# rteammco/super-resolution

Measured on AMD Instinct MI355X. Metric: MAP gradient iterations/sec at fixed HR size, higher is better.
Workload: dtype f64

## Files before the change

super-resolution_amd/csrc/kernels_ztile.hip:

```cpp


#include <type_traits>

#include "ztile_dev.hpp"

namespace srmap {

namespace {

template <typename T, int S, int B, int REGK, int R, bool WD, bool SP>
__global__ __launch_bounds__((ZCfg<T, S, B, REGK, R>::NT), (sizeof(T) == 4 || S == 2 ? 6 : 4)) void k_eval_z(
    ZArgs<T, B, ZCfg<T, S, B, REGK, R>::NP> A) {
  using C = ZCfg<T, S, B, REGK, R>;
  constexpr int HB = C::HB, NV = C::NV, RU = C::RU;
  constexpr int kBorderLds = (int)((16 * sizeof(int2) + kBorderTabEntries * sizeof(ZEntry) + 16 * sizeof(double) + sizeof(T) - 1) / sizeof(T));
  __shared__ T xs[C::XS_ELEMS > kBorderLds ? C::XS_ELEMS : kBorderLds];
  __shared__ T zs[C::ZS_ELEMS > 0 ? C::ZS_ELEMS : 1];
  __shared__ T cs[C::CS_ELEMS > 0 ? C::CS_ELEMS : 1];
  __shared__ double red[2][C::NW];
  __shared__ T wcs[32];
  __shared__ T whs[(C::RU > 0 ? C::RU : 1) * S * C::CW];

  {
    const T* a_x = A.x; const T* a_y = A.y; const T* a_w = A.w; T* a_g = A.g;
// ... 15 lines not shown
      if (WD && A.fold_xk != nullptr) border_block<T, S, B, C::NT, WD, WD>(A, Bd, bidx, blockIdx.z, xs, A.nby * gridDim.x);
      else border_block<T, S, B, C::NT, WD, false>(A, Bd, bidx, blockIdx.z, xs, A.nby * gridDim.x);
    }
    else if (threadIdx.x == 0) {
      const int nbb = A.nby * gridDim.x;
      put_partial<WD>(A, (size_t)A.n_tile_partials + (size_t)blockIdx.z * nbb + bidx, 0.0, 0.0);
    }
    return;
  }
  const int by = blockIdx.y - A.nby, nby_t = gridDim.y - A.nby;
  int tby = by, tbx = blockIdx.x;
  {
    const int q = gridDim.x >> 3, rem = gridDim.x & 7;
    const int n0 = blockIdx.x, nbot = (rem == 0) ? (int)gridDim.x - 1 : 8 * q - 1;
    const int n = (nbot > 1) ? (n0 == 1 ? nbot : (n0 == nbot ? 1 : n0)) : n0;
    const int bnd = n & 7;
    tby = bnd * q + (bnd < rem ? bnd : rem) + (n >> 3);
    tbx = (by == 0) ? 0 : (by == 1 ? nby_t - 1 : by - 1);
  }
  if (A.sel_mode != 0 && ((A.sel_mode == 1) != (tby >= A.sel0 && tby < A.sel1))) return;
  const int R0 = tby * C::TH, CJ0 = tbx * C::CW, C0 = CJ0 * S;
  const int ch = blockIdx.z;
  const size_t N = (size_t)A.W * A.H;
  const size_t nl = (size_t)A.wl * A.hl;
  const bool fold = WD && A.fold_xk != nullptr;
  const T* xplane = (fold ? A.fold_xk : A.x) + (size_t)ch * N;
  const int gr = R0 + wv;
  const int gc0 = C0 + S * lane;
  const int cellg = CJ0 + lane;
  const bool want_data = (A.terms & SRMAP_TERM_DATA) != 0;
  const bool want_reg = REGK != 0 && (A.terms & SRMAP_TERM_REG) != 0 && R0 >= A.rr0 && R0 < A.rr1;
  const T* ybase = A.y + (size_t)ch * nl;
  constexpr int ARI = (C::XR + C::NW - 1) / C::NW;
  constexpr int EXTRA = C::XC - C::CW;
  constexpr bool XT = ARI >= 2 && (C::NW - 1) + (ARI - 1) * C::NW >= C::XR && C::XR * EXTRA <= 64;
  T va[ARI][S], vb[ARI][S], ma[ARI], mb[ARI];
  T vda[WD ? ARI : 1][S], vdb[WD ? ARI : 1][S];
  bool owna[ARI] = {}, ownb[ARI] = {};
  size_t xoa[ARI] = {}, xob[ARI] = {};
#pragma unroll
  for (int it = 0; it < ARI; ++it) {
    const bool xt_slot = XT && it == ARI - 1 && wv == C::NW - 1;
    const int row = xt_slot ? lane / EXTRA : wv + it * C::NW;
    const int grr = R0 - C::HU + row;
    const bool row_in = row < C::XR && (unsigned)grr < (unsigned)A.H;
    const int gca = xt_slot ? CJ0 - C::XCL + C::CW + lane % EXTRA : CJ0 - C::XCL + lane, gcb = gca + C::CW;
    const bool ina = row_in && (unsigned)gca < (unsigned)A.wl;
    const bool inb = !XT && row_in && lane < EXTRA && (unsigned)gcb < (unsigned)A.wl;
    const T* sa = xplane + (ina ? (size_t)grr * A.W + (size_t)gca * S : (size_t)0);
    const T* sb = xplane + (inb ? (size_t)grr * A.W + (size_t)gcb * S : (size_t)0);
#pragma unroll
    for (int pc = 0; pc < S; ++pc) va[it][pc] = sa[pc];
    if (!XT) {
#pragma unroll
      for (int pc = 0; pc < S; ++pc) vb[it][pc] = sb[pc];
    }
    if (WD) {
#pragma unroll
      for (int pc = 0; pc < S; ++pc) { vda[it][pc] = T(0); vdb[it][pc] = T(0); }
      if (fold) {
        const T* dpl = A.dvec + (size_t)ch * N;
        const T* da = dpl + (sa - xplane);
        const T* db = dpl + (sb - xplane);
#pragma unroll
        for (int pc = 0; pc < S; ++pc) vda[it][pc] = da[pc];
        if (!XT) {
#pragma unroll
          for (int pc = 0; pc < S; ++pc) vdb[it][pc] = db[pc];
        }
        const int orow = row - C::HU;
        owna[it] = ina && orow >= 0 && orow < C::TH && gca >= CJ0 && gca < CJ0 + C::CW;
        ownb[it] = inb && orow >= 0 && orow < C::TH && gcb >= CJ0 && gcb < CJ0 + C::CW;
        xoa[it] = (size_t)grr * A.W + (size_t)gca * S;
        xob[it] = (size_t)grr * A.W + (size_t)gcb * S;
      }
    }
    ma[it] = ina ? Pre<T>::up(T(1)) : T(0);
    mb[it] = inb ? Pre<T>::up(T(1)) : T(0);
  }
  T ypre[NV];
#pragma unroll
  for (int v = 0; v < NV; ++v) ypre[v] = T(0);
  const int rm = A.E + HB + 1, cm = (A.E + HB + S) / S + 1;
  const bool edge = (R0 - rm < 0) || (R0 + C::TH + rm > A.H) || (CJ0 - cm < 0) || (CJ0 + C::CW + cm > A.wl) ||
                    A.cr0 > 0 || A.cr1 < A.H;
  const int hrowz = wv == 0 ? -HB : C::TH - 1 + HB;
  const bool has_z_halo = want_data && B > 1 && A.g != nullptr && wv < 2;
  T ypre2[NV];
#pragma unroll
  for (int v = 0; v < NV; ++v) ypre2[v] = T(0);
  if (!SP && want_data) z_row_prefetch<T, S, B, C>(A, wv, R0, CJ0, lane, edge, ybase, ypre);
  if (!SP && has_z_halo) z_row_prefetch<T, S, B, C>(A, hrowz, R0, CJ0, lane, edge, ybase, ypre2);
  const T* wplane = (want_reg && A.w) ? A.w + (size_t)ch * N : nullptr;
  T wreg[S];
#pragma unroll
  for (int pc = 0; pc < S; ++pc) wreg[pc] = T(1);
  if (wplane != nullptr && gr < A.H && gc0 < A.W) {
#pragma unroll
    for (int pc = 0; pc < S; ++pc) wreg[pc] = wplane[(size_t)gr * A.W + gc0 + pc];
  }
  const bool reg_halo_on = want_reg && A.g != nullptr && RU > 0;
  const int hrow = -(wv - 1);
  const bool has_reg_halo = reg_halo_on && wv >= 2 && wv < 2 + RU;
  T whalo[S];
#pragma unroll
  for (int pc = 0; pc < S; ++pc) whalo[pc] = T(1);
  if (has_reg_halo && wplane != nullptr && R0 + hrow >= 0 && gc0 < A.W) {
#pragma unroll
    for (int pc = 0; pc < S; ++pc) whalo[pc] = wplane[(size_t)(R0 + hrow) * A.W + gc0 + pc];
  }

  T wcolv = T(1);
  const bool col_task = reg_halo_on && (wv == 4 || wv == 5) && lane < C::TH + RU;
  if (col_task && wplane != nullptr) {
    const int hgr = R0 + lane - RU, hgc = C0 - (wv == 4 ? 1 : 2);
    if (hgr >= 0 && hgr < A.H && hgc >= 0) wcolv = wplane[(size_t)hgr * A.W + hgc];
  }

  const DirScale dsc = dir_scale(WD ? A.fold_norms : nullptr);
  if (WD && fold) {
    T* xout = A.fold_x + (size_t)ch * N;
#pragma unroll
    for (int it = 0; it < ARI; ++it) {
#pragma unroll
      for (int pc = 0; pc < S; ++pc) va[it][pc] = va[it][pc] + A.fold_stp * dir_elem<T>(vda[it][pc], dsc);
      if (owna[it]) {
#pragma unroll
        for (int pc = 0; pc < S; ++pc) xout[xoa[it] + pc] = va[it][pc];
      }
      if (!XT) {
#pragma unroll
        for (int pc = 0; pc < S; ++pc) vb[it][pc] = vb[it][pc] + A.fold_stp * dir_elem<T>(vdb[it][pc], dsc);
        if (ownb[it]) {
#pragma unroll
          for (int pc = 0; pc < S; ++pc) xout[xob[it] + pc] = vb[it][pc];
        }
      }
    }
  }
#pragma unroll
  for (int it = 0; it < ARI; ++it) {
    const bool xt_slot = XT && it == ARI - 1 && wv == C::NW - 1;
    if (xt_slot) {
      const int xrow = lane / EXTRA;
      if (xrow < C::XR) {
#pragma unroll
        for (int pc = 0; pc < S; ++pc) xs[xrow * C::XROW + pc * C::XC + C::CW + lane % EXTRA] = va[it][pc] * ma[it];
      }
      continue;
    }
    const int row = wv + it * C::NW;
    if (row < C::XR) {
#pragma unroll
      for (int pc = 0; pc < S; ++pc) xs[row * C::XROW + pc * C::XC + lane] = va[it][pc] * ma[it];
      if (!XT && lane < EXTRA) {
#pragma unroll
        for (int pc = 0; pc < S; ++pc) xs[row * C::XROW + pc * C::XC + C::CW + lane] = vb[it][pc] * mb[it];
      }
    }
  }
  if (col_task) wcs[(wv - 4) * 16 + lane] = wcolv;
  if (has_reg_halo) {
#pragma unroll
    for (int pc = 0; pc < S; ++pc) whs[((wv - 2) * S + pc) * C::CW + lane] = whalo[pc];
  }
  __syncthreads();

  T mk[S];
#pragma unroll
  for (int pc = 0; pc < S; ++pc) mk[pc] = (gr < A.H && gc0 + pc < A.W) ? T(1) : T(0);

  T acc[S], zown[S];
#pragma unroll
  for (int j = 0; j < S; ++j) { acc[j] = T(0); zown[j] = T(0); }
  double cost_data = 0.0, cost_reg = 0.0;

  auto phase1_data = [&]() __attribute__((always_inline)) {
  if (SP && want_data) {
    T dummy[S];
    const bool row_edge = (R0 - A.Dr - 2 * S < 0) || (R0 + C::TH + A.Dr + 2 * S > A.H);
    const int mj = A.Dr / S + 3;
    const bool col_inner = (CJ0 - mj >= 0) && (CJ0 + C::CW + mj <= A.wl);
    if (row_edge) {
      z_row_sp2<T, S, B, C, true, true>(A, zs, wv, R0, CJ0, lane, ch, zown);
      if (has_z_halo) z_row_sp2<T, S, B, C, true, true>(A, zs, hrowz, R0, CJ0, lane, ch, dummy);
    } else if (!col_inner) {
      z_row_sp2<T, S, B, C, false, true>(A, zs, wv, R0, CJ0, lane, ch, zown);
      if (has_z_halo) z_row_sp2<T, S, B, C, false, true>(A, zs, hrowz, R0, CJ0, lane, ch, dummy);
    } else {
      z_row_sp2<T, S, B, C, false, false>(A, zs, wv, R0, CJ0, lane, ch, zown);
      if (has_z_halo) z_row_sp2<T, S, B, C, false, false>(A, zs, hrowz, R0, CJ0, lane, ch, dummy);
    }
  }
  if (!SP && want_data) {
    T dummy[S];
    double dcost = 0.0;
    if (edge) {
      z_row<T, S, B, C, true>(A, xs, zs, wv, R0, CJ0, lane, ybase, true, ypre, true, mk, zown, cost_data);
      if (has_z_halo) z_row<T, S, B, C, true>(A, xs, zs, hrowz, R0, CJ0, lane, ybase, true, ypre2, false, mk, dummy, dcost);
    } else {
      z_row<T, S, B, C, false>(A, xs, zs, wv, R0, CJ0, lane, ybase, true, ypre, true, mk, zown, cost_data);
      if (has_z_halo) z_row<T, S, B, C, false>(A, xs, zs, hrowz, R0, CJ0, lane, ybase, true, ypre2, false, mk, dummy, dcost);
    }
  }
  };
  phase1_data();
  if (want_reg) {
    const bool reg_border = (R0 + C::TH + C::WIN > A.H) || (C0 + C::TW + C::WIN > A.W);
    const bool cost_row = gr >= A.cr0 && gr < A.cr1;
    if (reg_border)
      reg_row<T, S, REGK, R, C, true, true>(acc, cost_reg, xs, cs, wreg, wv, lane, gr, gc0, A.W, A.H, A.lambda, A.powtab, A.pwsum, cost_row);
    else
      reg_row<T, S, REGK, R, C, false, true>(acc, cost_reg, xs, cs, wreg, wv, lane, gr, gc0, A.W, A.H, A.lambda, A.powtab, A.pwsum, cost_row);
    if (has_reg_halo) {
      T dacc[S];
      double dc = 0.0;
      T whl[S];
#pragma unroll
      for (int pc = 0; pc < S; ++pc) whl[pc] = whs[((wv - 2) * S + pc) * C::CW + lane];
      if (C0 + C::TW + C::WIN > A.W || R0 + C::WIN > A.H)
        reg_row<T, S, REGK, R, C, true, false>(dacc, dc, xs, cs, whl, hrow, lane, R0 + hrow, gc0, A.W, A.H, A.lambda, A.powtab, A.pwsum, false);
      else
        reg_row<T, S, REGK, R, C, false, false>(dacc, dc, xs, cs, whl, hrow, lane, R0 + hrow, gc0, A.W, A.H, A.lambda, A.powtab, A.pwsum, false);
    }
    if (col_task) {
      const T wcol = wcs[(wv - 4) * 16 + lane];
      const int rowrel = lane - RU;
      const int lo = rowrel * C::XROW, lc = rowrel * C::CROW;
      if (reg_border) {
        if (RU >= 1 && wv == 4) reg_halo_col<T, S, REGK, R, C, -1, true>(xs + lo, cs + lc, wcol, rowrel, R0, C0, A.W, A.H, A.lambda, A.powtab);
        if (RU >= 2 && wv == 5) reg_halo_col<T, S, REGK, R, C, -2, true>(xs + lo, cs + lc, wcol, rowrel, R0, C0, A.W, A.H, A.lambda, A.powtab);
      } else {
        if (RU >= 1 && wv == 4) reg_halo_col<T, S, REGK, R, C, -1, false>(xs + lo, cs + lc, wcol, rowrel, R0, C0, A.W, A.H, A.lambda, A.powtab);
        if (RU >= 2 && wv == 5) reg_halo_col<T, S, REGK, R, C, -2, false>(xs + lo, cs + lc, wcol, rowrel, R0, C0, A.W, A.H, A.lambda, A.powtab);
      }
    }
  }
  __syncthreads();

  T dreg[S];
#pragma unroll
  for (int pc = 0; pc < S; ++pc) dreg[pc] = T(0);
  if (WD && gr < A.H && gc0 < A.W && gr >= A.cr0 && gr < A.cr1) {
    const T* dp = A.dvec + (size_t)ch * N + (size_t)gr * A.W + gc0;
#pragma unroll
    for (int pc = 0; pc < S; ++pc) dreg[pc] = dir_elem<T>(dp[pc], dsc);
  }
  if (want_data && A.g != nullptr) {
    const T sc = (T)(2 * S * S);
#pragma unroll
    for (int pc = 0; pc < S; ++pc) {
      T zz;
      if (B == 1) {
        zz = zown[pc];
      } else {
        zz = T(0);
#pragma unroll
        for (int a = 0; a < B; ++a) zz += k1_tap<B>(A, a) * zs[(wv + a) * C::ZROW + pc * C::CW + lane];
      }
      if (SP)
        zz = ((unsigned)(gr - A.Dr) < (unsigned)(A.H - 2 * A.Dr) && (unsigned)(gc0 + pc - A.Dr) < (unsigned)(A.W - 2 * A.Dr)) ? zz : T(0);
      acc[pc] += sc * zz;
    }
  }
  if (want_reg && A.g != nullptr) reg_pass2z<T, S, REGK, R, C>(acc, xs, cs, wv, lane, A.powtab);

  if (SP && want_data && A.g != nullptr && A.ringbuf != nullptr) {
    const int Dr = A.Dr;
    if (R0 < Dr || R0 + C::TH > A.H - Dr || C0 < Dr || C0 + C::TW > A.W - Dr) {
      const int band = Dr * A.W, mid = A.H - 2 * Dr;
      const T* rb = A.ringbuf + (size_t)ch * (size_t)(2 * band + 2 * Dr * mid);
#pragma unroll
      for (int pc = 0; pc < S; ++pc) {
        const int gc = gc0 + pc;
        if (gr < A.H && gc < A.W) {
          int t = -1;
          if (gr < Dr) t = gr * A.W + gc;
          else if (gr >= A.H - Dr) t = band + (gr - (A.H - Dr)) * A.W + gc;
          else if (gc < Dr) t = 2 * band + (gr - Dr) * 2 * Dr + gc;
          else if (gc >= A.W - Dr) t = 2 * band + (gr - Dr) * 2 * Dr + Dr + (gc - (A.W - Dr));
          if (t >= 0) acc[pc] += rb[t];
        }
      }
    }
  }
// ... 612 lines not shown
```

super-resolution_amd/csrc/ztile_dev.hpp:

```cpp
#pragma once
#include <algorithm>
#include <climits>
#include <cmath>
#include <cstdlib>
#include <vector>

#include "cg_norm.hpp"
#include "srmap_internal.hpp"

namespace srmap {

static inline int fdiv(int a, int b) { return (a >= 0) ? a / b : -((-a + b - 1) / b); }
static inline int pmod(int a, int b) { return a - fdiv(a, b) * b; }

namespace {

template <int CTRL>
__device__ __forceinline__ double dpp_perm_d(double v) {
  int lo = __double2loint(v), hi = __double2hiint(v);
  lo = __builtin_amdgcn_update_dpp(0, lo, CTRL, 0xf, 0xf, true);
  hi = __builtin_amdgcn_update_dpp(0, hi, CTRL, 0xf, 0xf, true);
  return __hiloint2double(hi, lo);
}
__device__ __forceinline__ double readlane_d(double v, int l) {
// ... 156 lines not shown
    __syncthreads();
    double t = 0.0;
    for (int i = 0; i < NT / 64; ++i) t += red[i];
    tot[pass] = t;
  }
  if (timed_out) {
    if (tid == 0) { A.cost_out[0] = __builtin_nan(""); A.cost_out[6] = 1.0; if (A.to_host != nullptr) *(volatile double*)A.to_host = 1.0; if (WD && A.pub != nullptr) { A.pub[0] = A.cost_out[0]; A.pub[1] = 0.0; __threadfence_system(); *(volatile double*)A.tag_slot = A.tag; } }
    return;
  }
  for (int i = tid; i < A.n_partials; i += NT) {
    st_agent(reinterpret_cast<unsigned long long*>(A.mpart) + i, kSentinel);
    if (WD) st_agent(reinterpret_cast<unsigned long long*>(A.mpart_gd) + i, kSentinel);
  }
  if (tid == 0) {
    const double v = tot[0];
    A.cost_out[0] = v;
    if (WD) {
      A.cost_out[1] = tot[1];
      if (A.pub != nullptr) {
        A.pub[0] = v;
        A.pub[1] = tot[1];
        __threadfence_system();
        *(volatile double*)A.tag_slot = A.tag;
      }
    }
  }
}

template <typename T> struct BorderArgs;

template <typename T, int B, int NP>
struct ZArgs {
  const T* x;
  const T* y;
  const T* w;
  T* g;
  int W, H, wl, hl;
  int nby;
  int E;
  int terms;
  int obs_C;
  int cr0, cr1;
  int rr0, rr1;
  int sel_mode, sel0, sel1;
  int n_tile_partials;
  int MS;
  int cntk[4][8];
  long long off0[4][4];
  T blur3[3];
  T k1s[2];
  T lambda;
  T powtab[NP];
  T pwsum;
  double* partials;
  const T* dvec;
  double* partials_gd;
  const BorderArgs<T>* bd;
  ZEntry aux0[4][4];
  const int* cnt;
  const long long* off;
  const ZEntry* aux;
  const T* rbuf;
  const ZSrc* spsrc;
  int spn[4];
  int spmax;
  int Dr;
  const T* ringbuf;
  RingRects ring;
  int mfinish;
  int n_partials;
  double* mpart;
  double* mpart_gd;
  double* cost_out;
  double* pub;
  double* tag_slot;
  double tag;
  double* to_host;
  const double* xpart;
  int n_xpart;
  const T* fold_xk;
  T* fold_x;
  T fold_stp;
  const double* fold_norms;
};

template <typename T> struct Pre;
template <> struct Pre<double> {
  static constexpr int Q = 512;
  static __device__ __forceinline__ double up(double v) { return __builtin_ldexp(v, Q); }
  static __device__ __forceinline__ double down(double v) { return __builtin_ldexp(v, -Q); }
};
template <> struct Pre<float> {
  static constexpr int Q = 64;
  static __device__ __forceinline__ float up(float v) { return __builtin_ldexpf(v, Q); }
  static __device__ __forceinline__ float down(float v) { return __builtin_ldexpf(v, -Q); }
};
template <typename T>
__device__ __forceinline__ T sgn_pre(T dq, T pw) { return __builtin_fmin(__builtin_fmax(dq, -pw), pw); }
template <>
__device__ __forceinline__ float sgn_pre<float>(float dq, float pw) { return __builtin_amdgcn_fmed3f(dq, -pw, pw); }
template <typename T>
__device__ __forceinline__ T step_pre(T dq) { return __builtin_fmin(__builtin_fmax(dq + T(0.5), T(0)), T(1)); }

template <typename C>
__device__ __forceinline__ constexpr int xi(int row, int col) {
  return row * C::XROW + posmod(col, C::TW / C::CW) * C::XC + C::XCL + floordiv(col, C::TW / C::CW);
}
template <typename C>
__device__ __forceinline__ constexpr int ci(int row, int col) {
  return row * C::CROW + posmod(col, C::TW / C::CW) * C::CC + C::CCL + floordiv(col, C::TW / C::CW);
}

template <typename U>
__device__ __forceinline__ U ctab(const U* p, size_t i) {
  typedef const U __attribute__((address_space(4))) * CP;
  return ((CP)(unsigned long long)p)[i];
}
__device__ __forceinline__ ZEntry ctab(const ZEntry* p, size_t i) {
  typedef const int __attribute__((address_space(4))) * CP;
  CP q = (CP)(unsigned long long)(p + i);
  ZEntry e;
  e.k = q[0]; e.io = q[1]; e.jo = q[2]; e.oyx = q[3];
  return e;
}

template <int B, typename ArgsT>
__device__ __forceinline__ auto blur_tap(const ArgsT& A, int a, int e) {
  if (B == 1) return A.blur3[2];
  const bool ca = a == (B - 1) / 2, ce = e == (B - 1) / 2;
  return (ca && ce) ? A.blur3[2] : ((ca || ce) ? A.blur3[1] : A.blur3[0]);
}
template <int B, typename ArgsT>
__device__ __forceinline__ auto k1_tap(const ArgsT& A, int a) { return (B == 1 || a == (B - 1) / 2) ? A.k1s[1] : A.k1s[0]; }

template <typename ArgsT>
__device__ __forceinline__ ZEntry aux0_at(const ArgsT& A, int pr, int pc) {
  ZEntry e;
  e.k = A.aux0[pr][pc].k; e.io = A.aux0[pr][pc].io; e.jo = A.aux0[pr][pc].jo; e.oyx = A.aux0[pr][pc].oyx;
  return e;
}

template <typename T>
__device__ __forceinline__ T obs_at(const T* __restrict__ yk, int i, int j, int hl, int wl) {
  const int ic = i < 0 ? 0 : (i >= hl ? hl - 1 : i);
  const int jc = j < 0 ? 0 : (j >= wl ? wl - 1 : j);
  return yk[(size_t)ic * wl + jc];
}

template <int S>
__device__ __forceinline__ void row_phase(int gr, int& rc, int& pr) {
  rc = (gr >= 0) ? gr / S : -((-gr + S - 1) / S);
  pr = gr - rc * S;
}

template <typename T, int S, typename C, bool EDGE, typename ArgsT>
__device__ __forceinline__ void load_obs_row(const ArgsT& A, int pr, int rc, int t, int cell0, int lane,
                                             const T* __restrict__ ybase, const int (&cn)[S], T (&yv)[C::NV]) {
  constexpr int HB = C::HB, NV = C::NV;
  const size_t slot = (size_t)(t * S + pr) * S;
  const T* yrow = ybase + ((long long)rc * A.wl + cell0);
  if (!EDGE) {
    long long offs[S];
#pragma unroll
    for (int pc = 0; pc < S; ++pc) offs[pc] = (t == 0) ? A.off0[pr][pc] : ctab(A.off, slot + pc);
#pragma unroll
    for (int v = 0; v < NV; ++v) {
      const int pcv = v - HB, pc = posmod(pcv, S), dc = floordiv(pcv, S);
      const T* yp = yrow + (offs[pc] + dc);
      yv[v] = yp[(unsigned)lane];
    }
    return;
  }
  ZEntry ent[S];
#pragma unroll
  for (int pc = 0; pc < S; ++pc) ent[pc] = (t == 0) ? aux0_at(A, pr, pc) : ctab(A.aux, slot + pc);
#pragma unroll
  for (int v = 0; v < NV; ++v) {
    const int pcv = v - HB, pc = posmod(pcv, S), dc = floordiv(pcv, S);
    const ZEntry e = ent[pc];
    yv[v] = obs_at<T>(ybase + (size_t)e.k * A.obs_C * ((size_t)A.wl * A.hl), rc + e.io, cell0 + lane + dc + e.jo, A.hl, A.wl);
  }
  (void)cn;
}

template <typename T, int S, int B, typename C, bool EDGE, typename ArgsT>
__device__ __forceinline__ void z_row(const ArgsT& A, const T* __restrict__ xs, T* __restrict__ zs, int rowrel,
                                      int R0, int cell0, int lane, const T* __restrict__ ybase, bool use_pre,
                                      const T (&ypre)[C::NV], bool count, const T (&mk)[S], T (&zout)[S],
                                      double& cost) {
  constexpr int HB = C::HB, NV = C::NV;
  int rc, pr;
  row_phase<S>(R0 + rowrel, rc, pr);
  const int xrow = rowrel + C::HU;
  T bx[NV], btop[NV], bleft[NV], bcorner[NV];
#pragma unroll
  for (int v = 0; v < NV; ++v) { bx[v] = T(0); btop[v] = T(0); bleft[v] = T(0); bcorner[v] = T(0); }
#pragma unroll
  for (int a = 0; a < B; ++a) {
    T xr[NV + B - 1];
#pragma unroll
    for (int j = 0; j < NV + B - 1; ++j) xr[j] = xs[xi<C>(xrow + a - HB, j - 2 * HB) + lane];
#pragma unroll
    for (int v = 0; v < NV; ++v) {
#pragma unroll
      for (int e = 0; e < B; ++e) bx[v] += blur_tap<B>(A, a, e) * xr[v + e];
      if (EDGE && B > 1) {
        bleft[v] += blur_tap<B>(A, a, 0) * xr[v];
        if (a == 0) {
#pragma unroll
          for (int e = 0; e < B; ++e) btop[v] += blur_tap<B>(A, 0, e) * xr[v + e];
          bcorner[v] = blur_tap<B>(A, 0, 0) * xr[v];
        }
      }
    }
  }
  const T unscale = Pre<T>::down(T(1));
  int cn[S];
#pragma unroll
  for (int pc = 0; pc < S; ++pc) cn[pc] = A.cntk[pr][pc];
  const int mmax = A.cntk[pr][S];
  const int mfull = EDGE ? 0 : A.cntk[pr][S + 1];
  T z[NV];
#pragma unroll
  for (int v = 0; v < NV; ++v) z[v] = T(0);
  for (int t = 0; t < mmax; ++t) {
    T yv[NV];
    if (t == 0 && use_pre) {
#pragma unroll
      for (int v = 0; v < NV; ++v) yv[v] = ypre[v];
    } else {
      load_obs_row<T, S, C, EDGE>(A, pr, rc, t, cell0, lane, ybase, cn, yv);
    }
    if (!EDGE && t < mfull) {
#pragma unroll
      for (int v = 0; v < NV; ++v) {
        const int pcv = v - HB;
        const T rr = bx[v] * unscale - yv[v];
        z[v] += rr;
        if (pcv >= 0 && pcv < S && count) cost += (double)rr * (double)rr;
      }
      continue;
    }
    const size_t slot = (size_t)(t * S + pr) * S;
#pragma unroll
    for (int v = 0; v < NV; ++v) {
      const int pcv = v - HB, pc = posmod(pcv, S), dc = floordiv(pcv, S);
      const bool own = pcv >= 0 && pcv < S;
      if (t < cn[pc]) {
        T rr;
        if (!EDGE) {
          rr = bx[v] * unscale - yv[v];
          z[v] += rr;
          if (own && count) cost += (double)rr * (double)rr;
        } else {
          const ZEntry e = (t == 0) ? aux0_at(A, pr, pc) : ctab(A.aux, slot + pc);
          const int i = rc + e.io, j = cell0 + lane + dc + e.jo;
          T bxv = bx[v];
          if (B > 1) {
            const bool j0 = j == 0;
            if (i == 0) bxv = bxv - btop[v] - (j0 ? bleft[v] - bcorner[v] : T(0));
            else bxv = bxv - (j0 ? bleft[v] : T(0));
          }
          rr = bxv * unscale - yv[v];
          rr = ((unsigned)i < (unsigned)A.hl && (unsigned)j < (unsigned)A.wl) ? rr : T(0);
          z[v] += rr;
          if (own && count && S * i >= A.cr0 && S * i < A.cr1) {
            const double rd = (double)(rr * mk[own ? pcv : 0]);
            cost += rd * (double)rr;
          }
        }
      }
    }
  }
  if (B == 1) {
#pragma unroll
    for (int pc = 0; pc < S; ++pc) zout[pc] = z[pc];
  } else {
#pragma unroll
    for (int pc = 0; pc < S; ++pc) {
      T zh = T(0);
#pragma unroll
      for (int e = 0; e < B; ++e) zh += k1_tap<B>(A, e) * z[pc + e];
      zs[(rowrel + HB) * C::ZROW + pc * C::CW + lane] = zh;
    }
  }
}

constexpr int kSpChunk = 4;
template <typename T, int S, typename C, int A, bool COLCLAMP, typename ArgsT>
__device__ __forceinline__ void sp_apply(const ArgsT& A_, const T (&rv)[kSpSlots(S, C::HB)], int elo, int jbase, int lane,
                                         T w0, T w1, T (&z)[C::NV]) {
  constexpr int HB = C::HB, NSL = kSpSlots(S, C::HB);
  constexpr int ELO = ((A - S >= -HB) || (A - 1 - S >= -HB)) ? -1 : 0;
  (void)elo;
#pragma unroll
  for (int sl = 0; sl < NSL; ++sl) {
    const int e = ELO + sl;
    if (e > 1) continue;
    const int p0 = A + S * e, p1 = A - 1 + S * e;
    const bool in0 = p0 >= -HB && p0 < S + HB, in1 = p1 >= -HB && p1 < S + HB;
    if (!in0 && !in1) continue;
    T m0 = w0, m1 = w1;
    if (COLCLAMP) {
      const bool ok = (unsigned)(jbase + lane + e) < (unsigned)A_.wl;
      m0 = ok ? w0 : T(0);
      m1 = ok ? w1 : T(0);
    }
    if (in0) z[(in0 ? p0 : 0) + HB] += m0 * rv[sl];
    if (in1) z[(in1 ? p1 : 0) + HB] += m1 * rv[sl];
  }
}

template <typename T, int S, int B, typename C, bool EDGE, bool COLCLAMP, typename ArgsT>
__device__ __forceinline__ void z_row_sp2(const ArgsT& A, T* __restrict__ zs, int rowrel, int R0, int cell0, int lane, int ch,
                                          T (&zout)[S]) {
  constexpr int HB = C::HB, NV = C::NV, NSL = kSpSlots(S, C::HB);
  int rc, pr;
  row_phase<S>(R0 + rowrel, rc, pr);
  const size_t nl = (size_t)A.wl * A.hl;
  const int ns = A.spn[pr];
  T z[NV];
#pragma unroll
  for (int v = 0; v < NV; ++v) z[v] = T(0);
  typedef const ZSrc __attribute__((address_space(4))) * SrcPtr;
  SrcPtr tab = (SrcPtr)(unsigned long long)(A.spsrc + (size_t)pr * A.spmax);
  for (int n0 = 0; n0 < ns; n0 += kSpChunk) {
    int rk[kSpChunk], rio[kSpChunk], rq[kSpChunk], ram[kSpChunk];
    double rw0[kSpChunk], rw1[kSpChunk];
#pragma unroll
    for (int c = 0; c < kSpChunk; ++c) {
      rk[c] = tab[n0 + c].k; rio[c] = tab[n0 + c].io; rq[c] = tab[n0 + c].q; ram[c] = tab[n0 + c].am;
      rw0[c] = tab[n0 + c].w0; rw1[c] = tab[n0 + c].w1;
    }
    T rv[kSpChunk][NSL];
    int as[kSpChunk], jb[kSpChunk];
#pragma unroll
    for (int c = 0; c < kSpChunk; ++c) {
      const int i = rc + rio[c];
      as[c] = ram[c] & 0xff;
      if (EDGE && (unsigned)i >= (unsigned)A.hl) as[c] = kSpNull;
      jb[c] = cell0 + rq[c];
      const int elo = (ram[c] >> 8) - 1;
      const bool live = as[c] != kSpNull;
      const T* base = A.rbuf + (size_t)((live ? rk[c] : 0) * A.obs_C + ch) * nl;
      const unsigned rowoff = live ? (unsigned)i * (unsigned)A.wl : 0u;
#pragma unroll
      for (int sl = 0; sl < NSL; ++sl) {
        if (!COLCLAMP) {
          rv[c][sl] = base[rowoff + (unsigned)(live ? jb[c] + elo + sl + lane : 0)];
        } else {
          const int j = jb[c] + lane + elo + sl;
          rv[c][sl] = base[rowoff + (unsigned)(live ? (j < 0 ? 0 : (j >= A.wl ? A.wl - 1 : j)) : 0)];
        }
      }
    }
#pragma unroll
    for (int c = 0; c < kSpChunk; ++c) {
      const int a = as[c];
      const int elo = (ram[c] >> 8) - 1;
      const T w0 = (T)rw0[c], w1 = (T)rw1[c];
      if (a == 0) sp_apply<T, S, C, 0, COLCLAMP>(A, rv[c], elo, jb[c], lane, w0, w1, z);
      else if (a == 1) sp_apply<T, S, C, 1, COLCLAMP>(A, rv[c], elo, jb[c], lane, w0, w1, z);
      else if (a == 2) sp_apply<T, S, C, (S > 2 ? 2 : 0), COLCLAMP>(A, rv[c], elo, jb[c], lane, w0, w1, z);
      else if (a == 3) sp_apply<T, S, C, (S > 3 ? 3 : 0), COLCLAMP>(A, rv[c], elo, jb[c], lane, w0, w1, z);
    }
  }
  if (B == 1) {
#pragma unroll
    for (int pc = 0; pc < S; ++pc) zout[pc] = z[pc];
  } else {
#pragma unroll
    for (int pc = 0; pc < S; ++pc) {
      T zh = T(0);
#pragma unroll
      for (int e = 0; e < B; ++e) zh += k1_tap<B>(A, e) * z[pc + e];
      zs[(rowrel + HB) * C::ZROW + pc * C::CW + lane] = zh;
    }
  }
}

template <typename T, int S, int B, typename C, typename ArgsT>
__device__ __forceinline__ void z_row_prefetch(const ArgsT& A, int rowrel, int R0, int cell0, int lane, bool edge,
                                               const T* __restrict__ ybase, T (&ypre)[C::NV]) {
  int rc, pr;
  row_phase<S>(R0 + rowrel, rc, pr);
  int cn[S];
#pragma unroll
  for (int pc = 0; pc < S; ++pc) cn[pc] = A.cntk[pr][pc];
  if (edge) load_obs_row<T, S, C, true>(A, pr, rc, 0, cell0, lane, ybase, cn, ypre);
  else load_obs_row<T, S, C, false>(A, pr, rc, 0, cell0, lane, ybase, cn, ypre);
}

template <typename T, int S, int REGK, int R, typename C, bool BORDER, bool FULL>
__device__ __forceinline__ void reg_row(T (&acc)[S], double& cost, const T* __restrict__ xs, T* __restrict__ cs,
                                        const T (&wv)[S], int rowrel, int lane, int gr, int gc0, int W, int H,
                                        T lambda, const T (&pw)[C::NP], T pwsum, bool cost_row) {
  constexpr int WIN = C::WIN;
  constexpr int NC = S + WIN;
  const int xrow = rowrel + C::HU;
  T x0v[S], rv[S], dv[S];
#pragma unroll
  for (int pc = 0; pc < S; ++pc) { rv[pc] = T(0); dv[pc] = T(0); }
  static_assert(S - 1 + WIN < 3 * S, "a window tap reaches at most two cells beyond the thread's own");
  const T mR1 = (!BORDER || gc0 + S < W) ? T(1) : T(0), mR2 = (!BORDER || gc0 + 2 * S < W) ? T(1) : T(0);
#pragma unroll
  for (int i = 0; i <= WIN; ++i) {
    if (BORDER && REGK == 2 && i > 0 && gr + i >= H) {
      if (FULL && sizeof(T) == 8 && i < R) {
#pragma unroll
        for (int pc = 0; pc < S; ++pc) {
#pragma unroll
          for (int j = 0; j < R; ++j) dv[pc] += pw[i + j] * T(0.5);
        }
      }
      continue;
    }
    T row[NC];
#pragma unroll
    for (int j = 0; j < NC; ++j) row[j] = xs[xi<C>(xrow + i, j) + lane];
    if (i == 0) {
#pragma unroll
      for (int pc = 0; pc < S; ++pc) x0v[pc] = row[pc];
    }
#pragma unroll
    for (int pc = 0; pc < S; ++pc) {
      if (REGK == 2) {
#pragma unroll
        for (int j = 0; j <= R; ++j) {
          if (i == 0 && j == 0) continue;
          T d = x0v[pc] - row[pc + j];
          if (BORDER && pc + j >= S) d = d * ((pc + j) / S == 1 ? mR1 : mR2);
          rv[pc] += pw[i + j] * absv(d);
          if (FULL && i < R && j < R) {
            if (sizeof(T) == 8) dv[pc] += pw[i + j] * step_pre<T>(d);
            else dv[pc] += sgn_pre<T>(d, pw[i + j]);
          }
        }
      } else if (i == 1) {
        T dyv = row[pc] - x0v[pc];
        if (BORDER) dyv = (gr + 1 < H) ? dyv : T(0);
        rv[pc] = absv(dyv) + rv[pc];
        if (FULL) dv[pc] = dv[pc] - sgn_pre<T>(dyv, T(1));
      } else {
        T dxv = row[pc + 1] - x0v[pc];
        if (BORDER) dxv = (gc0 + pc + 1 < W) ? dxv : T(0);
        rv[pc] = absv(dxv);
        if (FULL) dv[pc] = -sgn_pre<T>(dxv, T(1));
      }
    }
    pin(rv);
    if (FULL) pin(dv);
  }
#pragma unroll
  for (int pc = 0; pc < S; ++pc) {
    const T r = Pre<T>::down(rv[pc]);
    const T c = lambda * wv[pc];
    T cr2 = T(2) * c * r;
    const bool in_img = (unsigned)gr < (unsigned)H && (unsigned)(gc0 + pc) < (unsigned)W;
    if (FULL) {
      if (REGK == 2 && sizeof(T) == 8) dv[pc] = T(2) * dv[pc] - pwsum;
      acc[pc] += cr2 * dv[pc];
      const double cd = (in_img && cost_row) ? (double)c * (double)r * (double)r : 0.0;
      cost += cd;
    }
    if (!in_img || (REGK == 2 && gr == 0 && gc0 + pc == 0)) cr2 = T(0);
    cs[ci<C>(rowrel + C::RU, pc) + lane] = cr2;
  }
}

template <typename T, int S, int REGK, int R, typename C, int COL, bool BORDER>
__device__ __forceinline__ void reg_halo_col(const T* __restrict__ xs, T* __restrict__ cs, const T wt,
                                             int rowrel, int R0, int C0, int W, int H, T lambda,
                                             const T (&pw)[C::NP]) {
// ... 182 lines not shown
        }
      }
      corr *= (T)(2 * S * S);
      if (WD && qr >= A.cr0 && qr < A.cr1) gdc = -(double)corr * (double)dir_elem<T>(A.dvec[(size_t)ch * N + (size_t)qr * A.W + qc], ds);
    }
    if (A.g != nullptr) Bd.corr[(size_t)ch * Bd.n_ring + t] = corr;
  }
  {
    double v = cost;
#pragma unroll
    for (int o = 32; o > 0; o >>= 1) v += __shfl_down(v, o, 64);
    const int lane = tid & 63, wid = tid >> 6;
    if (lane == 0) red[wid] = v;
    __syncthreads();
    if (tid == 0) {
      double sum = 0.0;
      for (int i = 0; i < NT / 64; ++i) sum += red[i];
      if (!WD) put_partial<false>(A, (size_t)A.n_tile_partials + (size_t)ch * nbb + bidx, (double)(S * S) * sum, 0.0);
      else red[NT / 64] = (double)(S * S) * sum;
    }
    if (WD) {
      double w2 = gdc;
#pragma unroll
      for (int o = 32; o > 0; o >>= 1) w2 += __shfl_down(w2, o, 64);
      __syncthreads();
      if (lane == 0) red[wid] = w2;
      __syncthreads();
      if (tid == 0) {
        double sum = 0.0;
        for (int i = 0; i < NT / 64; ++i) sum += red[i];
        put_partial<true>(A, (size_t)A.n_tile_partials + (size_t)ch * nbb + bidx, red[NT / 64], sum);
      }
    }
  }
}


}

struct ZPlan {
  int S = 0, B = 1;
  int regk = 0, regr = 0, reg_index = -1;
  bool subpix = false;
  int Dr = 0;
  void* d_ringbuf = nullptr;
  ZSrc* d_spsrc = nullptr;
  int spn[4] = {0, 0, 0, 0};
  int spmax = 0;
  SpForwardPlan spf;
  int E = 0;
  int MS = 1;
  int n_ent = 0;
  int2* d_hdr = nullptr;
  ZEntry* d_ent = nullptr;
  int h_cnt[32] = {0};
  long long h_off0[16] = {0};
  ZEntry h_aux0[16] = {};
  int* d_cnt = nullptr;
  long long* d_off = nullptr;
  ZEntry* d_aux = nullptr;
  int n_ring = 0;
  RingRects ring = {{0, 0, 0, 0, 0, 0}};
  void* d_corr = nullptr;
  void* d_bd = nullptr;
  double* d_mpart = nullptr;
  size_t mpart_cap = 0;
};


struct MFin { bool on, publish; const double* xpart; int n_xpart; };

template <typename T, int S, int B, int REGK, int R>
static void fill_zargs(ZArgs<T, B, ZCfg<T, S, B, REGK, R>::NP>& A, srmap_problem* p, const Geometry& geo, int obs_c0,
                       unsigned terms, const T* x, T* g, const T* wts, const ZPlan& z, double* partials, const T* dvec,
                       double* partials_gd) {
  using C = ZCfg<T, S, B, REGK, R>;
  A.x = x; A.y = (const T*)p->d_obs + (size_t)obs_c0 * geo.w * geo.h; A.w = wts; A.g = g; A.partials = partials;
  A.dvec = dvec; A.partials_gd = partials_gd;
  A.cnt = z.d_cnt; A.off = z.d_off; A.aux = z.d_aux; A.MS = z.MS;
  A.spsrc = z.d_spsrc; A.spmax = z.spmax;
  for (int pr = 0; pr < 4; ++pr) A.spn[pr] = z.spn[pr];
  for (int pr = 0; pr < 4; ++pr) {
    for (int i = 0; i < 8; ++i) A.cntk[pr][i] = z.h_cnt[pr * 8 + i];
    for (int pc = 0; pc < 4; ++pc) { A.off0[pr][pc] = z.h_off0[pr * 4 + pc]; A.aux0[pr][pc] = z.h_aux0[pr * 4 + pc]; }
  }
  A.W = geo.W; A.H = geo.H; A.wl = geo.w; A.hl = geo.h;
  A.obs_C = p->geo.C;
  A.E = z.E;
  A.ring = z.ring;
  A.cr0 = geo.cr0; A.cr1 = geo.cr1;
  A.rr0 = geo.rr0; A.rr1 = geo.rr1;
  A.terms = (int)terms;
  if (B == 1) { A.blur3[0] = A.blur3[1] = A.blur3[2] = T(1); A.k1s[0] = A.k1s[1] = T(1); }
  else {
    const int hb = (B - 1) / 2;
    A.blur3[0] = (T)p->blur2d[0]; A.blur3[1] = (T)p->blur2d[hb]; A.blur3[2] = (T)p->blur2d[hb * B + hb];
    A.k1s[0] = (T)p->blur1d[0]; A.k1s[1] = (T)p->blur1d[hb];
  }
  A.lambda = T(0);
  for (int i = 0; i < C::NP; ++i) A.powtab[i] = T(1);
  if (REGK != 0) {
    const RegSpec& rs = p->reg[z.reg_index];
    A.lambda = (T)rs.lambda;
    if (REGK == 2) for (int i = 0; i < C::NP; ++i) A.powtab[i] = (T)rs.pow_table[i];
  }
  A.pwsum = T(0);
  if (REGK == 2)
    for (int i = 0; i < R; ++i)
      for (int j = 0; j < R; ++j)
        if (i + j > 0) A.pwsum += A.powtab[i + j];
  A.fold_xk = nullptr; A.fold_x = nullptr; A.fold_stp = T(0); A.fold_norms = nullptr;
}

}
```

Baseline: 23350.

## Add column-edge specialization for z residual rows in the tiled kernel

Splits the previous single edge flag into row-edge and column-edge cases. Tiles that touch only the left or right border now take a cheaper column path that clamps column indices and masks out-of-range cells, and applies the blur correction only on the left side, instead of the fully general edge path. Kernel arguments are read straight from the kernarg segment for this path. The cost is extra template instantiations, higher code size and register pressure, and a new jo0 field in the argument struct.

```diff
diff --git a/super-resolution_amd/csrc/kernels_ztile.hip b/super-resolution_amd/csrc/kernels_ztile.hip
--- a/super-resolution_amd/csrc/kernels_ztile.hip
+++ b/super-resolution_amd/csrc/kernels_ztile.hip
@@ -121,15 +121,19 @@
 #pragma unroll
   for (int v = 0; v < NV; ++v) ypre[v] = T(0);
   const int rm = A.E + HB + 1, cm = (A.E + HB + S) / S + 1;
-  const bool edge = (R0 - rm < 0) || (R0 + C::TH + rm > A.H) || (CJ0 - cm < 0) || (CJ0 + C::CW + cm > A.wl) ||
-                    A.cr0 > 0 || A.cr1 < A.H;
+  const bool row_edge = (R0 - rm < 0) || (R0 + C::TH + rm > A.H) || A.cr0 > 0 || A.cr1 < A.H;
+  const bool col_left = CJ0 - cm < 0, col_right = CJ0 + C::CW + cm > A.wl;
+  constexpr int ZCOL = kColumnClass<T, S, B, WD> ? Z_COLUMN : Z_FULL;
+  const int zmode = row_edge ? Z_FULL : ((col_left || col_right) ? ZCOL : Z_INTERIOR);
+  typedef const ZArgs<T, B, C::NP> __attribute__((address_space(4))) * KArgs;
+  const auto& AK = *(KArgs)__builtin_amdgcn_kernarg_segment_ptr();
   const int hrowz = wv == 0 ? -HB : C::TH - 1 + HB;
   const bool has_z_halo = want_data && B > 1 && A.g != nullptr && wv < 2;
   T ypre2[NV];
 #pragma unroll
   for (int v = 0; v < NV; ++v) ypre2[v] = T(0);
-  if (!SP && want_data) z_row_prefetch<T, S, B, C>(A, wv, R0, CJ0, lane, edge, ybase, ypre);
-  if (!SP && has_z_halo) z_row_prefetch<T, S, B, C>(A, hrowz, R0, CJ0, lane, edge, ybase, ypre2);
+  if (!SP && want_data) z_row_prefetch<T, S, B, C, ZCOL>(A, AK, wv, R0, CJ0, lane, zmode, ybase, ypre);
+  if (!SP && has_z_halo) z_row_prefetch<T, S, B, C, ZCOL>(A, AK, hrowz, R0, CJ0, lane, zmode, ybase, ypre2);
   const T* wplane = (want_reg && A.w) ? A.w + (size_t)ch * N : nullptr;
   T wreg[S];
 #pragma unroll
@@ -234,12 +238,15 @@
   if (!SP && want_data) {
     T dummy[S];
     double dcost = 0.0;
-    if (edge) {
-      z_row<T, S, B, C, true>(A, xs, zs, wv, R0, CJ0, lane, ybase, true, ypre, true, mk, zown, cost_data);
-      if (has_z_halo) z_row<T, S, B, C, true>(A, xs, zs, hrowz, R0, CJ0, lane, ybase, true, ypre2, false, mk, dummy, dcost);
+    if (zmode == Z_FULL) {
+      z_row<T, S, B, C, Z_FULL>(A, xs, zs, wv, R0, CJ0, lane, ybase, true, ypre, true, false, mk, zown, cost_data);
+      if (has_z_halo) z_row<T, S, B, C, Z_FULL>(A, xs, zs, hrowz, R0, CJ0, lane, ybase, true, ypre2, false, false, mk, dummy, dcost);
+    } else if (zmode == Z_COLUMN) {
+      z_row<T, S, B, C, Z_COLUMN>(AK, xs, zs, wv, R0, CJ0, lane, ybase, true, ypre, true, col_left, mk, zown, cost_data);
+      if (has_z_halo) z_row<T, S, B, C, Z_COLUMN>(AK, xs, zs, hrowz, R0, CJ0, lane, ybase, true, ypre2, false, col_left, mk, dummy, dcost);
     } else {
-      z_row<T, S, B, C, false>(A, xs, zs, wv, R0, CJ0, lane, ybase, true, ypre, true, mk, zown, cost_data);
-      if (has_z_halo) z_row<T, S, B, C, false>(A, xs, zs, hrowz, R0, CJ0, lane, ybase, true, ypre2, false, mk, dummy, dcost);
+      z_row<T, S, B, C, Z_INTERIOR>(A, xs, zs, wv, R0, CJ0, lane, ybase, true, ypre, true, false, mk, zown, cost_data);
+      if (has_z_halo) z_row<T, S, B, C, Z_INTERIOR>(A, xs, zs, hrowz, R0, CJ0, lane, ybase, true, ypre2, false, false, mk, dummy, dcost);
     }
   }
   };
diff --git a/super-resolution_amd/csrc/ztile_dev.hpp b/super-resolution_amd/csrc/ztile_dev.hpp
--- a/super-resolution_amd/csrc/ztile_dev.hpp
+++ b/super-resolution_amd/csrc/ztile_dev.hpp
@@ -262,6 +262,7 @@
   T* fold_x;
   T fold_stp;
   const double* fold_norms;
+  int jo0[4][4];
 };
 
 template <typename T> struct Pre;
@@ -333,13 +334,46 @@
   pr = gr - rc * S;
 }
 
-template <typename T, int S, typename C, bool EDGE, typename ArgsT>
+enum ZMode : int { Z_INTERIOR = 0, Z_FULL = 1, Z_COLUMN = 2 };
+template <typename T, int S, int B, bool WD>
+constexpr bool kColumnClass = !(sizeof(T) == 8 && B == 3 && (S == 2 || (S == 3 && WD)));
+
+template <int S> struct ZColRow { long long rowoff[S]; int jo[S]; };
+template <int S, typename ArgsT>
+__device__ __forceinline__ ZColRow<S> col_row(const ArgsT& A, int pr, int t) {
+  ZColRow<S> r;
+  if (t == 0) {
+#pragma unroll
+    for (int pc = 0; pc < S; ++pc) { r.jo[pc] = A.jo0[pr][pc]; r.rowoff[pc] = A.off0[pr][pc] - r.jo[pc]; }
+  } else {
+    const size_t slot = (size_t)(t * S + pr) * S;
+    const long long* off = A.off;
+    const ZEntry* aux = A.aux;
+#pragma unroll
+    for (int pc = 0; pc < S; ++pc) { r.jo[pc] = ctab(aux, slot + pc).jo; r.rowoff[pc] = ctab(off, slot + pc) - r.jo[pc]; }
+  }
+  return r;
+}
+template <typename T, int S, typename C>
+__device__ __forceinline__ void load_obs_col(const ZColRow<S>& r, const T* __restrict__ yr0, int wl, int cell0, int lane,
+                                             T (&yv)[C::NV]) {
+  constexpr int HB = C::HB, NV = C::NV;
+#pragma unroll
+  for (int v = 0; v < NV; ++v) {
+    const int pcv = v - HB, pc = posmod(pcv, S), dc = floordiv(pcv, S);
+    const T* yp = yr0 + r.rowoff[pc];
+    const int j = cell0 + lane + dc + r.jo[pc];
+    yv[v] = yp[(unsigned)(j < 0 ? 0 : (j >= wl ? wl - 1 : j))];
+  }
+}
+
+template <typename T, int S, typename C, int MODE, typename ArgsT>
 __device__ __forceinline__ void load_obs_row(const ArgsT& A, int pr, int rc, int t, int cell0, int lane,
                                              const T* __restrict__ ybase, const int (&cn)[S], T (&yv)[C::NV]) {
   constexpr int HB = C::HB, NV = C::NV;
   const size_t slot = (size_t)(t * S + pr) * S;
   const T* yrow = ybase + ((long long)rc * A.wl + cell0);
-  if (!EDGE) {
+  if (MODE == Z_INTERIOR) {
     long long offs[S];
 #pragma unroll
     for (int pc = 0; pc < S; ++pc) offs[pc] = (t == 0) ? A.off0[pr][pc] : ctab(A.off, slot + pc);
@@ -351,6 +385,11 @@
     }
     return;
   }
+  if (MODE == Z_COLUMN) {
+    const int wl = A.wl;
+    load_obs_col<T, S, C>(col_row<S>(A, pr, t), ybase + (long long)rc * wl, wl, cell0, lane, yv);
+    return;
+  }
   ZEntry ent[S];
 #pragma unroll
   for (int pc = 0; pc < S; ++pc) ent[pc] = (t == 0) ? aux0_at(A, pr, pc) : ctab(A.aux, slot + pc);
@@ -363,12 +402,56 @@
   (void)cn;
 }
 
-template <typename T, int S, int B, typename C, bool EDGE, typename ArgsT>
+
+template <typename T, int S, int B, typename C, bool LEFT, typename ArgsT>
+__device__ __forceinline__ void z_rounds_col(const ArgsT& A, const T* __restrict__ xs, int xrow, int pr, int rc, int cell0,
+                                             int lane, const T* __restrict__ ybase, bool use_pre, const T (&ypre)[C::NV],
+                                             bool count, const T (&mk)[S], const int (&cn)[S], int mmax,
+                                             const T (&bx)[C::NV], T (&z)[C::NV], double& cost) {
+  constexpr int HB = C::HB, NV = C::NV;
+  const T unscale = Pre<T>::down(T(1));
+  const int wl = A.wl;
+  for (int t = 0; t < mmax; ++t) {
+    const ZColRow<S> row = col_row<S>(A, pr, t);
+    T yv[NV];
+    if (t == 0 && use_pre) {
+#pragma unroll
+      for (int v = 0; v < NV; ++v) yv[v] = ypre[v];
+    } else {
+      load_obs_col<T, S, C>(row, ybase + (long long)rc * wl, wl, cell0, lane, yv);
+    }
+#pragma unroll
+    for (int v = 0; v < NV; ++v) {
+      const int pcv = v - HB, pc = posmod(pcv, S), dc = floordiv(pcv, S);
+      const bool own = pcv >= 0 && pcv < S;
+      if (t < cn[pc]) {
+        const int j = cell0 + lane + dc + row.jo[pc];
+        T bxv = bx[v];
+        if (B > 1 && LEFT) {
+          T bl = T(0);
+#pragma unroll
+          for (int a = 0; a < B; ++a) bl += blur_tap<B>(A, a, 0) * xs[xi<C>(xrow + a - HB, v - 2 * HB) + lane];
+          bxv = bxv - (j == 0 ? bl : T(0));
+        }
+        T rr = bxv * unscale - yv[v];
+        rr = ((unsigned)j < (unsigned)wl) ? rr : T(0);
+        z[v] += rr;
+        if (own && count) {
+          const double rd = (double)(rr * mk[own ? pcv : 0]);
+          cost += rd * (double)rr;
+        }
+      }
+    }
+  }
+}
+
+template <typename T, int S, int B, typename C, int MODE, typename ArgsT>
 __device__ __forceinline__ void z_row(const ArgsT& A, const T* __restrict__ xs, T* __restrict__ zs, int rowrel,
                                       int R0, int cell0, int lane, const T* __restrict__ ybase, bool use_pre,
-                                      const T (&ypre)[C::NV], bool count, const T (&mk)[S], T (&zout)[S],
+                                      const T (&ypre)[C::NV], bool count, bool left, const T (&mk)[S], T (&zout)[S],
                                       double& cost) {
   constexpr int HB = C::HB, NV = C::NV;
+  constexpr bool EDGE = MODE == Z_FULL;
   int rc, pr;
   row_phase<S>(R0 + rowrel, rc, pr);
   const int xrow = rowrel + C::HU;
@@ -398,20 +481,27 @@
   int cn[S];
 #pragma unroll
   for (int pc = 0; pc < S; ++pc) cn[pc] = A.cntk[pr][pc];
-  const int mmax = A.cntk[pr][S];
-  const int mfull = EDGE ? 0 : A.cntk[pr][S + 1];
+  const int mall = A.cntk[pr][S];
+  const int mmax = MODE == Z_COLUMN ? 0 : mall;
+  const int mfull = MODE != Z_INTERIOR ? 0 : A.cntk[pr][S + 1];
   T z[NV];
 #pragma unroll
   for (int v = 0; v < NV; ++v) z[v] = T(0);
+  if (MODE == Z_COLUMN) {
+    if (B > 1 && left)
+      z_rounds_col<T, S, B, C, true>(A, xs, xrow, pr, rc, cell0, lane, ybase, use_pre, ypre, count, mk, cn, mall, bx, z, cost);
+    else
+      z_rounds_col<T, S, B, C, false>(A, xs, xrow, pr, rc, cell0, lane, ybase, use_pre, ypre, count, mk, cn, mall, bx, z, cost);
+  }
   for (int t = 0; t < mmax; ++t) {
     T yv[NV];
     if (t == 0 && use_pre) {
 #pragma unroll
       for (int v = 0; v < NV; ++v) yv[v] = ypre[v];
     } else {
-      load_obs_row<T, S, C, EDGE>(A, pr, rc, t, cell0, lane, ybase, cn, yv);
-    }
-    if (!EDGE && t < mfull) {
+      load_obs_row<T, S, C, MODE>(A, pr, rc, t, cell0, lane, ybase, cn, yv);
+    }
+    if (MODE == Z_INTERIOR && t < mfull) {
 #pragma unroll
       for (int v = 0; v < NV; ++v) {
         const int pcv = v - HB;
@@ -559,16 +649,17 @@
   }
 }
 
-template <typename T, int S, int B, typename C, typename ArgsT>
-__device__ __forceinline__ void z_row_prefetch(const ArgsT& A, int rowrel, int R0, int cell0, int lane, bool edge,
-                                               const T* __restrict__ ybase, T (&ypre)[C::NV]) {
+template <typename T, int S, int B, typename C, int ZCOL, typename ArgsT, typename KArgsT>
+__device__ __forceinline__ void z_row_prefetch(const ArgsT& A, const KArgsT& AK, int rowrel, int R0, int cell0, int lane,
+                                               int zmode, const T* __restrict__ ybase, T (&ypre)[C::NV]) {
   int rc, pr;
   row_phase<S>(R0 + rowrel, rc, pr);
   int cn[S];
 #pragma unroll
   for (int pc = 0; pc < S; ++pc) cn[pc] = A.cntk[pr][pc];
-  if (edge) load_obs_row<T, S, C, true>(A, pr, rc, 0, cell0, lane, ybase, cn, ypre);
-  else load_obs_row<T, S, C, false>(A, pr, rc, 0, cell0, lane, ybase, cn, ypre);
+  if (zmode == Z_FULL) load_obs_row<T, S, C, Z_FULL>(A, pr, rc, 0, cell0, lane, ybase, cn, ypre);
+  else if (ZCOL == Z_COLUMN && zmode == Z_COLUMN) load_obs_row<T, S, C, Z_COLUMN>(AK, pr, rc, 0, cell0, lane, ybase, cn, ypre);
+  else load_obs_row<T, S, C, Z_INTERIOR>(A, pr, rc, 0, cell0, lane, ybase, cn, ypre);
 }
 
 template <typename T, int S, int REGK, int R, typename C, bool BORDER, bool FULL>
@@ -917,7 +1008,7 @@
   for (int pr = 0; pr < 4; ++pr) A.spn[pr] = z.spn[pr];
   for (int pr = 0; pr < 4; ++pr) {
     for (int i = 0; i < 8; ++i) A.cntk[pr][i] = z.h_cnt[pr * 8 + i];
-    for (int pc = 0; pc < 4; ++pc) { A.off0[pr][pc] = z.h_off0[pr * 4 + pc]; A.aux0[pr][pc] = z.h_aux0[pr * 4 + pc]; }
+    for (int pc = 0; pc < 4; ++pc) { A.off0[pr][pc] = z.h_off0[pr * 4 + pc]; A.aux0[pr][pc] = z.h_aux0[pr * 4 + pc]; A.jo0[pr][pc] = z.h_aux0[pr * 4 + pc].jo; }
   }
   A.W = geo.W; A.H = geo.H; A.wl = geo.w; A.hl = geo.h;
   A.obs_C = p->geo.C;
```

Result: slower. 23000 (-1.5%).
